# YannisLamp/crypto-recommendation

Hardware: AMD Instinct MI355X
Metric: point hash+assign ops/sec at d=128, N=10M, K=256; 1/2/4/8 MI355X (higher is better)
Workload: dtype fp32 points; split-f16 MFMA scores (f32 accumulate); tuples, bucket IDs and cluster IDs bit-exact (x87-exact hashing, certified argmin); distances: certified f32, <= 2^-20 relative to the reference's fp64 (north star: 1e-5; the context's default LSHKM_DIST_CERTIFIED mode), LSHKM_DIST_EXACT for the r; 1 GPU; C3 Lloyd K=256 + C2 LSH L=5 k=4 hashing, N=10000000 per GPU, d=128; N_per_gpu=10000000, N_total=10000000, d=128, K=256, L=5, k=4, nb=100000, parallelism=dp1 (row shards)

## Files before the change

### crypto-recommendation_amd/csrc/api.cpp

```cpp
#include <hip/hip_runtime.h>

#include <algorithm>
#include <cmath>
#include <cstring>
#include <map>
#include <mutex>
#include <random>
#include <sstream>
#include <string>
#include <vector>

#include "../../include/lshkm.h"
#include "common.h"
#include "kernels.h"
#include "index.h"

namespace lshkm {
static thread_local std::string g_err;
void set_error(const std::string& msg) { g_err = msg; }

int device_cu_count(int* ncu) {
    static std::mutex mu;
    static std::map<int, int> cus;
    int dev = 0;
// ... 551 lines not shown
    return lsh_hash_impl(lsh, X, N, tuples, phi, bucket);
}

int lshkm_lsh_hash_f64(lshkm_lsh lsh, const double* X, int64_t N, int32_t* tuples, int32_t* phi, int32_t* bucket) {
    return lsh_hash_impl(lsh, X, N, tuples, phi, bucket);
}

}

static int assign_path(int metric, int d, int K, bool f64) {
    if (test_switch("LSHKM_ASSIGN_PATH", "exact")) return 2;
    if (!test_switch("LSHKM_ASSIGN_PATH", "f32")) {
        const FusedRoute r = fused_route(metric != LSHKM_METRIC_EUCLIDEAN, f64, d, K, false, 0, 0,
                                         test_switch("LSHKM_FUSED_FORM", "chunked"));
        if (r.form != FusedForm::none) return r.rows == 0 ? 0 : 3;
    }
    return assign_dp(d) > 0 ? 1 : 2;
}

static bool fuse_hash(const lshkm_lsh_s* lsh, int metric, int K, bool f64) {
    const lshkm::ProjTable& pj = lsh->proj;
    if (lsh->metric != metric || !(metric == LSHKM_METRIC_EUCLIDEAN ? pj.fused_ok : pj.mfma_ok)) return false;
    return fused_route(metric != LSHKM_METRIC_EUCLIDEAN, f64, pj.d, K, true, pj.k, pj.LK,
                       test_switch("LSHKM_FUSED_FORM", "chunked")).form != FusedForm::none;
}

bool lshkm::exact_pruned(Pts X, int d, int K, int metric) {
    return K <= 1024 && d <= 256 && !test_switch("LSHKM_EXACT_PASS", "full") &&
           (metric == LSHKM_METRIC_EUCLIDEAN || !X.f64);
}

static size_t exact_ct_bytes(const AssignJob& q) { return (size_t)q.d * ((q.K + 255) / 256 * 256) * 8; }

int lshkm::exact_listed_prep(lshkm_ctx ctx, const AssignJob& q) {
    int rc;
    if ((rc = ctx->ws_ct.reserve(exact_ct_bytes(q)))) return rc;
    return launch_assign_pruned_prep(ctx->stream, q.X.f64, q.d, q.C, q.K, (float*)ctx->ws_ct.p,
                                     q.metric == LSHKM_METRIC_EUCLIDEAN ? 0 : 1);
}

int lshkm::exact_listed(lshkm_ctx ctx, const AssignJob& q, const RowList& l, bool exact_dist, bool prepped,
                        const double* xn2, const double* nbv) {
    const bool prune = exact_pruned(q.X, q.d, q.K, q.metric);
    if (!prune && (q.metric != LSHKM_METRIC_EUCLIDEAN || (l.nseg == 0 && q.d > 256)))
        return launch_assign_exact(ctx->stream, q, l, xn2, nbv);
    int rc;
    if ((rc = ctx->ws_ct.reserve(exact_ct_bytes(q)))) return rc;
    if (prune) return launch_assign_pruned_list(ctx->stream, q, (float*)ctx->ws_ct.p, l, exact_dist ? 1 : 0, prepped);
    return launch_assign_exact_list(ctx->stream, q, (double*)ctx->ws_ct.p, l);
}

static int assign_f32_mfma(lshkm_ctx ctx, const AssignJob& q) {
    hipStream_t s = ctx->stream;
    const int DP = assign_dp(q.d), Kpad = (q.K + 63) / 64 * 64;
    const int64_t N = q.N;
    int rc;
    if ((rc = ctx->ws_c32.reserve((size_t)Kpad * DP * 4)) || (rc = ctx->ws_cconst.reserve((size_t)3 * Kpad * 4)) ||
        (rc = ctx->ws_ambig.reserve((size_t)std::max<int64_t>(N, 1) * 2 * 4)) ||
        (rc = ctx->ws_counter.reserve(64)))
        return rc;
    unsigned long long* cnt = (unsigned long long*)ctx->ws_counter.p;
    LSHKM_HIP(hipMemsetAsync(cnt, 0, 16, s));
    if ((rc = launch_centroid_prep(s, q.C, q.K, Kpad, q.d, DP, q.metric, q.X.f64, (float*)ctx->ws_c32.p, (float*)ctx->ws_cconst.p))) return rc;
    if ((rc = launch_assign_mfma(s, q.X, N, q.d, DP, q.C, q.K, Kpad, q.metric, (const float*)ctx->ws_c32.p, (const float*)ctx->ws_cconst.p,
                                 q.assign, q.dist, (int32_t*)ctx->ws_ambig.p, cnt))) return rc;
    RowList l;
// ... 225 lines not shown
```

### crypto-recommendation_amd/csrc/fused.hip

```cpp
#include "../../include/lshkm.h"
#include "fused_impl.h"
#include "index.h"

namespace lshkm {

namespace {

struct FusedPlan {
    bool hash = false, cos = false;
    int rows = 0;
    int nblk = 0;
    int64_t seg_rows = 0;
    int np_hi = 0;
    int np_refine = 0;
};

int fused_workspace(lshkm_ctx ctx, const FusedShape& sh, FusedWorkspace& w) {
    const FusedLayout l = fused_layout(sh);
    int rc;
    struct { Buf& b; size_t bytes; } const bufs[] = {
        {ctx->ws_c32, l.c16},      {ctx->ws_cconst, l.cconst}, {ctx->ws_ambig, l.list1}, {ctx->ws_counter, l.counter},
        {ctx->ws_seg, l.seg1},     {ctx->ws_hfix, l.fix},      {ctx->ws_seg3, l.seg3},   {ctx->ws_part, l.part},
        {ctx->ws_ambig2, l.list2}, {ctx->ws_seg2, l.seg2},     {ctx->ws_tuples, l.tuples}, {ctx->ws_cf32, l.cf32},
        {ctx->ws_c64p, l.c64p},    {ctx->ws_xn2, l.xn2}};
    for (const auto& e : bufs)
        if (e.bytes && (rc = e.b.reserve(e.bytes))) return rc;
    const auto at = [](const Buf& b, size_t off) { return off == FusedLayout::NONE ? nullptr : (char*)b.p + off; };
    w.list_cap = l.list_cap;
    w.Ch = (_Float16*)at(ctx->ws_c32, 0); w.Cl = (_Float16*)at(ctx->ws_c32, l.cl_off);
    w.cbound = (float*)at(ctx->ws_cconst, 0); w.cnh = (float*)at(ctx->ws_cconst, l.cnh_off);
    w.nbv = (double*)at(ctx->ws_cconst, l.nbv_off);
    if (l.cf32) { w.C32 = (float*)at(ctx->ws_cf32, 0); w.rn32 = (float*)at(ctx->ws_cf32, l.rn32_off); }
    if (l.c64p) w.C64p = ctx->ws_c64p.as<double>();
    w.list1 = ctx->ws_ambig.as<int32_t>(); w.seg1 = ctx->ws_seg.as<int32_t>();
    w.list2 = ctx->ws_ambig2.as<int32_t>(); w.seg2 = ctx->ws_seg2.as<int32_t>();
    if (l.seg3) w.seg3 = ctx->ws_seg3.as<int32_t>();
    w.hfix = (unsigned long long*)at(ctx->ws_hfix, l.hfix_off);
    w.cfix = (unsigned long long*)at(ctx->ws_hfix, l.cfix_off);
    w.hfix2 = (unsigned long long*)at(ctx->ws_hfix, l.hfix2_off);
    if (l.part) w.part = ctx->ws_part.as<float4>();
    w.cnt = ctx->ws_counter.as<unsigned long long>();
    if (l.xn2) w.xn2 = ctx->ws_xn2.as<double>();
    if (l.tuples) w.tuples = ctx->ws_tuples.as<int32_t>();
    return 0;
}

FusedArgs fused_common_args(lshkm_ctx ctx, const AssignRequest& q, const FusedShape& sh, const FusedWorkspace& w) {
    FusedArgs a{};
    a.X = q.X.f64 ? nullptr : q.X.f(); a.X64 = q.X.f64 ? q.X.d() : nullptr;
    a.N = q.N; a.d = q.d;
    a.xvec = sh.rows == 1 ? (a.d % 4 == 0 && ((uintptr_t)a.X & 15) == 0) : (a.d % 2 == 0 && ((uintptr_t)a.X64 & 15) == 0);
    a.Ch = w.Ch; a.Cl = w.Cl; a.cnh = w.cnh; a.cbound = w.cbound; a.Kpad = sh.Kpad();
    a.C64 = w.C64p ? w.C64p : q.C; a.Cd = q.C;
    a.C32 = w.C32; a.rn32 = w.rn32; a.fast_dist = sh.fast ? 1 : 0;
    a.assign = q.assign; a.dist = q.dist;
    a.stats = ctx->stats.as<unsigned long long>();
    a.nb = 1;
    if (q.lsh) {
        const ProjTable& pj = q.lsh->proj;
        a.Vh = pj.vh_d.as<_Float16>(); a.Vl = pj.vl_d.as<_Float16>(); a.PT = pj.PT_d.as<double>();
        a.tv = pj.t_d.as<float>(); a.pnorm = pj.pn_d.as<double>(); a.v1 = pj.v1_d.as<double>();
        a.rv = pj.r_d.as<int32_t>(); a.w = pj.w; a.L = pj.L; a.k = pj.k; a.LK = pj.LK; a.LKpad = pj.LKpad;
        a.nb = q.lsh->nb;
    }
    a.bdiv = make_bucket_div(a.nb);
    if (sh.cosine) { a.nbv = w.nbv; a.xn2 = w.xn2; }
    a.cfix = w.cfix; a.cfix_counts = w.seg3; a.cfix_count = w.cfix ? w.cnt + CNT_CFIX : nullptr;
    a.pass_first = 1; a.pass_last = 1;
    return a;
}

void hash_outputs(FusedArgs& a, const AssignRequest& q, const FusedShape& sh, const FusedWorkspace& w) {
    a.hfix = w.hfix; a.hfix_count = w.hfix ? w.cnt + CNT_HFIX : nullptr;
    if (!q.lsh) return;
    a.phi = q.phi; a.bucket = q.bucket;
    a.tuples = sh.cosine ? nullptr : q.tuples ? q.tuples : w.tuples;
}

template <typename T>
// ... 69 lines not shown
            c->tev_side = true;
        }
        if (hipEventRecord(c->join_ev, c->side_stream) != hipSuccess) return kstatus("fused_assign (join)");
        return 0;
    }
    int join() {
        if (!open) return 0;
        if (hipStreamWaitEvent(c->stream, c->join_ev, 0) != hipSuccess) return kstatus("fused_assign (join)");
        open = false;
        return 0;
    }
    ~SideFork() { if (open) (void)hipStreamSynchronize(c->side_stream); }
};

#ifdef LSHKM_PHASE_TIMING
struct PhaseReport {
    hipStream_t s;
    unsigned long long* d = nullptr;
    explicit PhaseReport(hipStream_t s_) : s(s_) {
        static unsigned long long* prof_d = nullptr;
        if (!prof_d) (void)hipMalloc(&prof_d, 64);
        (void)hipMemsetAsync(prof_d, 0, 64, s);
        d = prof_d;
    }
    ~PhaseReport() {
        unsigned long long v[6];
        (void)hipMemcpyAsync(v, d, 48, hipMemcpyDeviceToHost, s);
        (void)hipStreamSynchronize(s);
        fprintf(stderr, "PHASES %llu %llu %llu %llu %llu\n", v[0], v[1], v[2], v[3], v[4]);
    }
};
#endif

}

int fused_assign(lshkm_ctx ctx, const AssignRequest& q) {
    hipStream_t s = ctx->stream;
    const bool cosine = q.metric != LSHKM_METRIC_EUCLIDEAN;
    const ProjTable* pj = q.lsh ? &q.lsh->proj : nullptr;
    const FusedRoute route = fused_route(cosine, q.X.f64, q.d, q.K, pj != nullptr, pj ? pj->k : 0, pj ? pj->LK : 0,
                                         test_switch("LSHKM_FUSED_FORM", "chunked"));
    if (route.form == FusedForm::none || (pj && (q.lsh->metric != q.metric || !pj->mfma_ok))) {
        set_error("fused_assign: no fused form runs this shape (fused_route, fused_layout.h)");
        return LSHKM_ERR_ARG;
    }
    FusedShape sh;
    sh.N = q.N; sh.d = q.d; sh.K = q.K; sh.cosine = cosine; sh.rows = route.rows;
    sh.hash = pj != nullptr; sh.LK = pj ? pj->LK : 0;
    sh.fast = !cosine && sh.rows != 2 && !q.force_exact && ctx->dist_mode == LSHKM_DIST_CERTIFIED;
    sh.image32 = sh.fast || (!cosine && sh.rows != 2 && sh.Kpad() <= 256 && !test_switch("LSHKM_GATHER32", "0"));
    sh.own_tuples = sh.hash && !cosine && !q.tuples;
    const bool pwfix = sh.pwfix();
    int rc;
    FusedWorkspace w;
    if ((rc = fused_workspace(ctx, sh, w))) return rc;
    LSHKM_HIP(hipMemsetAsync(w.cnt, 0, FUSED_COUNTER_CLEAR, s));
    if (ctx->timing) LSHKM_HIP(hipEventRecord(ctx->tev[0], s));
    ctx->tev_side = false;
    if ((rc = launch_fused_prep(s, q.C, q.K, q.d, cosine ? 1 : 0, w))) return rc;
    const bool xprep = exact_pruned(q.X, q.d, q.K, q.metric);
    if (xprep && (rc = exact_listed_prep(ctx, q))) return rc;
    if (w.xn2 && (rc = launch_row_sumsq(s, q.X.d(), q.N, q.d, w.xn2))) return rc;

    const FusedArgs common = fused_common_args(ctx, q, sh, w);
    RowList exact_rows;
    exact_rows.p = w.list1; exact_rows.count = w.cnt + CNT_AMBIG; exact_rows.bound = q.N;
    RecList dist_fix[2];
    int ndist_fix = 0;
    SideFork side{ctx};
    if (q.N > 0 && route.form == FusedForm::chunked) {
        FusedArgs a = common;
        hash_outputs(a, q, sh, w);
        a.ambig = w.list1; a.ambig_count = w.cnt + CNT_AMBIG;
        if ((rc = launch_fused_chunked(s, sh.hash, a))) return rc;
    } else if (q.N > 0) {
        FusedPlan p;
        p.hash = sh.hash; p.cos = cosine; p.rows = sh.rows;
        int ncu = 0;
        if (device_cu_count(&ncu)) return LSHKM_ERR_HIP;
        p.nblk = fused_grid(q.N, ncu);
        p.seg_rows = fused_seg_rows(q.N, p.nblk);
        if (p.nblk > FUSED_MAX_SEGS) {
            set_error("fused_assign: more blocks than list segments");
            return LSHKM_ERR_ARG;
        }
        p.np_hi = (sh.Kpad() + FH_KMAX - 1) / FH_KMAX;
        p.np_refine = (sh.Kpad() + FP_KMAX - 1) / FP_KMAX;
        const RowList l1 = segmented(w.list1, w.cnt + CNT_REFINED, w.seg1, q, p);
        const RecList lh = segmented(w.hfix, w.cnt + CNT_HFIX, w.seg1, q, p);
        const RowList l2 = segmented(w.list2, w.cnt + CNT_AMBIG, w.seg2, q, p);
        FusedArgs seg = common;
        seg.seg_rows = p.seg_rows; seg.part = w.part;
#ifdef LSHKM_PHASE_TIMING
        PhaseReport report(s);
        seg.prof = report.d;
#endif
        FusedArgs hi = seg;
        hash_outputs(hi, q, sh, w);
        hi.ambig = l1.p; hi.ambig_count = l1.count; hi.seg_counts = l1.counts;
        if ((rc = fused_hi_passes(s, hi, p))) return rc;
        if (sh.hash) {
            const bool forked = ctx->side_init() == 0;
            if (forked && (rc = side.fork())) return rc;
            launch_hash_fixup(forked ? ctx->side_stream : s, lh, cosine, hi);
            if (forked && (rc = side.end_side())) return rc;
        }
        FusedArgs rf = seg;
        rf.list_in = l1.p; rf.list_counts = l1.counts; rf.list_seg_rows = l1.seg_rows;
        rf.ambig = l2.p; rf.ambig_count = l2.count; rf.seg_counts = l2.counts;
        rf.hfix = cosine ? w.hfix2 : hi.hfix; rf.hfix_count = cosine ? w.cnt + CNT_CFIX : hi.hfix_count;
        if ((rc = fused_refine_passes(s, rf, p))) return rc;
        if (cosine && (rc = side.join())) return rc;
        if ((rc = kstatus("fused_hi_kernel"))) return rc;
        exact_rows = l2;
        if (cosine || pwfix) dist_fix[ndist_fix++] = segmented(w.cfix, w.cnt + CNT_CFIX, w.seg3, q, p);
        if (cosine) dist_fix[ndist_fix++] = segmented(w.hfix2, w.cnt + CNT_CFIX, w.seg2, q, p);
    }
    if (ctx->timing) LSHKM_HIP(hipEventRecord(ctx->tev[1], s));
    if ((rc = exact_listed(ctx, q, exact_rows, !sh.fast, xprep, cosine ? w.xn2 : nullptr, cosine ? w.nbv : nullptr)))
        return rc;
    if ((rc = side.join())) return rc;
    {
        int di[3], n = 0;
        const unsigned long long* sp[3];
        di[n] = STAT_REFINED; sp[n++] = w.cnt + CNT_REFINED;
        if (sh.hash) { di[n] = STAT_HASH_FIX; sp[n++] = w.cnt + CNT_HFIX; }
        di[n] = STAT_ASSIGN_AMBIG; sp[n++] = w.cnt + CNT_AMBIG;
        if ((rc = launch_add_counters(s, ctx->stats.as<unsigned long long>(), n, di, sp))) return rc;
    }
    if (cosine || pwfix) {
        if ((rc = launch_cos_fix_seg(s, q, ndist_fix, dist_fix, cosine ? w.xn2 : nullptr, cosine ? w.nbv : nullptr)))
            return rc;
        if ((rc = launch_add_counter(s, ctx->stats.as<unsigned long long>() + (cosine ? STAT_COS_FIX : STAT_POW_FIX),
                                     w.cnt + CNT_CFIX)))
            return rc;
    }
    return 0;
}

}
```

### crypto-recommendation_amd/csrc/fused_hi.hip

```cpp
#include "fused_impl.h"

namespace lshkm {

__host__ __device__ constexpr int fh_lds_bytes(int Kpad, bool hash) {
    return 16 + Kpad * FU_RS * 2 + Kpad * 4 + (hash ? 2 * 32 * FU_RS * 2 + FP_HC_BYTES : 0);
}
static_assert(fh_lds_bytes(FH_KMAX, true) <= 160 * 1024, "hi-only LDS image exceeds 160 KiB");
constexpr double FH_A = 130.0 * 0x1p-23;

constexpr int FH_WAVES_MPFAST = 12;
constexpr int FH_FAST_WAVES = 8;
template <bool HASH, bool MP, int MET, bool FAST = false>
__host__ __device__ constexpr int fh_waves() {
    return HASH && MP ? 12 : (MP && FAST ? FH_WAVES_MPFAST : (FAST && !MP ? FH_FAST_WAVES : 8));
}

__device__ inline int cosine_halves_finish(double sh0, double sl0, double ts0, double sh, double sl, double ts,
                                           double xa, double nbv, double& v) {
    const double mb = 2.0 * sqrt(__dmul_rn(xa, nbv)) * (1.0 + 0x1p-40);
    const double tsum = __dadd_rn(ts0, ts);
    if (!(tsum >= 0x1p-790)) return 2;
    IpAcc ip;
    const double t = __dadd_rn(sh0, sh);
    const double bb = __dsub_rn(t, sh0);
// ... 118 lines not shown
}

#ifndef LSHKM_ROWPF
#define LSHKM_ROWPF 3
#endif
constexpr int FH_ROWPF = LSHKM_ROWPF;
constexpr int FH_ROWPF_KMAX = 256;
constexpr int FH_ROWPF_WAVE = 32 * 64 * 4;
__host__ __device__ constexpr int fh_rowpf_off(int Kpad, bool hash) { return (fh_lds_bytes(Kpad, hash) + 255) & ~255; }
static_assert(fh_rowpf_off(FH_ROWPF_KMAX, true) + FH_FAST_WAVES * FH_ROWPF_WAVE <= 160 * 1024,
              "row prefetch buffers exceed 160 KiB");
static_assert(FH_ROWPF_KMAX <= FH_GATH_KMAX, "the FAST single-pass form runs where the gather ring would (fused.hip)");

__device__ inline void glds16s(const void* sbase, uint32_t voff, uint32_t lds_base, int lds_off) {
    unsigned keep;
    asm volatile("s_mov_b32 %0, m0\n\ts_add_u32 m0, %3, %4\n\ts_nop 0\n\tglobal_load_lds_dwordx4 %1, %2\n\ts_mov_b32 m0, %0"
                 : "=&s"(keep) : "v"(voff), "s"(sbase), "s"(lds_base), "n"(lds_off) : "memory", "scc");
}

template <bool HASH, bool MP = false, int MET = 0, int NIMG = 1, bool GATH = false, int ROWS = 0, bool FAST = false,
          int PF = 0, int HG = 4>
__global__ __launch_bounds__((64 * fh_waves<HASH, MP, MET, FAST>()), 1) void fused_hi_kernel(FusedArgs a) {
    constexpr int FH_WAVES = fh_waves<HASH, MP, MET, FAST>();
    constexpr int FH_THREADS = 64 * FH_WAVES;
    static_assert(NIMG == 1 || (!MP && MET == 0), "two-image form: euclidean, single launch");
    static_assert(!GATH || (!MP && MET == 0 && NIMG == 1 && FH_WAVES == 8), "gather ring: euclidean single pass");
    static_assert(ROWS == 0 || (!HASH && !MP && NIMG == 1), "general rows: Lloyd without hashing, one pass");
    static_assert(!(GATH && ROWS == 2), "fp64 rows re-read x in the chain: register loads of the winner rows");
    static_assert(!FAST || (MET == 0 && ROWS != 2 && NIMG == 1 && !GATH), "fast distance: euclidean, fp32 rows");
    static_assert(PF == 0 || (FAST && !MP && ROWS == 0 && FH_WAVES == FH_FAST_WAVES), "row prefetch: the FAST single-pass form");
    static_assert(HG == 4 || (HASH && MET == 0 && PF != 0 && HG >= 1 && HG < 4), "fewer live hash groups: the prefetching FAST form");
    constexpr bool PFR = (PF & 1) != 0, PFL = (PF & 2) != 0;
    extern __shared__ __attribute__((aligned(16))) char smem[];
    const int Kpad = a.Kpad;
    const bool fastd = FAST || a.fast_dist != 0;
    const int KI = NIMG == 2 ? FH_KMAX : Kpad;
    int* lcount = reinterpret_cast<int*>(smem);
    _Float16* lch = reinterpret_cast<_Float16*>(smem + 16);
    float* lcn = reinterpret_cast<float*>(lch + KI * FU_RS);
    _Float16* lvh = reinterpret_cast<_Float16*>(lcn + KI);
    _Float16* lvl = lvh + 32 * FU_RS;
    float* lpn0 = reinterpret_cast<float*>(lvl + 32 * FU_RS);
    float* lv10 = lpn0 + 32;
    float* lt0 = lv10 + 32;
    int32_t* lr0 = reinterpret_cast<int32_t*>(lt0 + 32);

    auto load_image = [&](int img) {
        const int r0 = img * KI, nr = NIMG == 2 && img == 1 ? Kpad - FH_KMAX : KI;
        constexpr int FH_CU = 8;
        for (int e0 = 0; e0 < nr * 16; e0 += FH_THREADS * FH_CU) {
            float4 v[FH_CU];
#pragma unroll
            for (int u = 0; u < FH_CU; u++) {
                const int e = e0 + u * FH_THREADS + (int)threadIdx.x < nr * 16 ? e0 + u * FH_THREADS + (int)threadIdx.x : 0;
                v[u] = *reinterpret_cast<const float4*>(a.Ch + (size_t)(r0 + (e >> 4)) * FU_D + (e & 15) * 8);
            }
#pragma unroll
            for (int u = 0; u < FH_CU; u++) {
                const int e = e0 + u * FH_THREADS + (int)threadIdx.x < nr * 16 ? e0 + u * FH_THREADS + (int)threadIdx.x : 0;
                *reinterpret_cast<float4*>(lch + (e >> 4) * FU_RS + (e & 15) * 8) = v[u];
            }
        }
        for (int e = threadIdx.x; e < nr; e += FH_THREADS) lcn[e] = a.cnh[r0 + e];
    };
    load_image(0);
    if (threadIdx.x < 3) lcount[threadIdx.x] = 0;
// ... 516 lines not shown
                }
                acc = take_from_upper(acc);
            }
            const bool pw_hard = pwl == nullptr && (pw.hard() || (ROWS != 2 && (__float_as_uint(a.cbound[7]) & 2u) != 0u));
            const int pw_other = __shfl_xor((int)pw_hard, 32);
            const bool hard = pw_hard || pw_other != 0;
            if (h == 1 && valid && cert) {
                a.assign[row] = I1;
                if (!hard) a.dist[row] = sqrt(acc);
            }
            const unsigned long long pb = __ballot(h == 1 && valid && cert && hard);
            if (pb) {
                const int leader = __builtin_ctzll(pb);
                int base = 0;
                if (lane == leader) base = atomicAdd(lcount + 2, __popcll(pb));
                base = __shfl(base, leader);
                if (h == 1 && valid && cert && hard) cfix_seg[base + __popcll(pb & ((1ull << lane) - 1ull))] = (unsigned long long)row;
            }
            __builtin_amdgcn_s_setprio(0);
        }
        PT_MARK(2)
    };
    if constexpr (PFR) {
        for (int64_t tile = tfirst + wave; tile < ntiles; tile += 2 * tstride) {
            tile_body(tile, xua, xub);
            if (tile + tstride >= ntiles) break;
            tile_body(tile + tstride, xub, xua);
        }
    } else {
        for (int64_t tile = tfirst + wave; NIMG == 2 ? rd < nround : tile < ntiles; tile += tstride, rd++)
            tile_body(tile, xua, xub);
    }
    PT_FLUSH
    __syncthreads();
    if (threadIdx.x < 2 && (!MP || (threadIdx.x == 0 ? (!HASH && a.pass_last != 0) : (HASH && a.pass_first)))) {
        const int c = lcount[threadIdx.x];
        a.seg_counts[SEG_SLOTS * blockIdx.x + threadIdx.x] = c;
        if (c) atomicAdd(threadIdx.x == 0 ? a.ambig_count : a.hfix_count, (unsigned long long)c);
    }
    if ((MET == 1 || !fastd) && threadIdx.x == 2 && (!MP || (!HASH && a.pass_last))) {
        const int c = lcount[2];
        a.cfix_counts[SEG_SLOTS * blockIdx.x + SEG_FIX] = c;
        if (c) atomicAdd(a.cfix_count, (unsigned long long)c);
    }
}

template <bool HASH, bool MP, int MET, int NIMG, bool GATH, int ROWS, bool FAST, int PF, int HG>
static void hi_launch(hipStream_t s, unsigned nblk, size_t lds, const FusedArgs& a) {
    hipLaunchKernelGGL((fused_hi_kernel<HASH, MP, MET, NIMG, GATH, ROWS, FAST, PF, HG>), dim3(nblk),
                       dim3(64 * fh_waves<HASH, MP, MET, FAST>()), lds, s, a);
}

int launch_fused_hi_pass(hipStream_t s, unsigned nblk, const HiForm& f, FusedArgs a) {
    size_t lds = (size_t)fh_lds_bytes(f.two_image ? FH_KMAX : a.Kpad, f.hash);
    a.pw_lds = 0;
    if (f.gath) {
        if (a.Kpad > FH_GATH_KMAX) {
            set_error("launch_fused_hi_pass: the gather ring needs K <= 256");
            return -1;
        }
        lds = (size_t)fh_gath_off(a.Kpad, f.hash) + 8 * FH_GATH_WAVE;
    } else if (f.rows == 2 && f.metric == 0) {
        constexpr int PW_BYTES = fh_waves<false, false, 0>() * 512 * 8;
        const size_t off = (lds + 255) & ~(size_t)255;
        if (off + PW_BYTES <= 160 * 1024) {
            a.pw_lds = (int)off;
// ... 54 lines not shown
```

### crypto-recommendation_amd/csrc/fused_impl.h

```cpp
#pragma once
#include <algorithm>
#include <cstdlib>
#include <cstring>
#include <cstdio>
#include <type_traits>

#include "common.h"
#include "kernels.h"
#include "hash_exact.h"
#include "exact.h"
#include "hash_tile.h"
#include "fused_args.h"

namespace lshkm {

static_assert(FU_D == FUSED_DIMS, "fused_layout.h states the kernels' dimension");
constexpr int FP_THREADS = 64 * FP_WAVES;
constexpr int FH_GATH_KMAX = 256;
constexpr int FP_HC_BYTES = 32 * (4 + 4 + 4 + 4);
constexpr int MFMA_PRIO = 1;
constexpr int CHAIN_PRIO = 2;

struct FusedWorkspace {
    int64_t list_cap = 0;
    _Float16 *Ch = nullptr, *Cl = nullptr;
    float *cbound = nullptr, *cnh = nullptr;
    double* nbv = nullptr;
    float *C32 = nullptr, *rn32 = nullptr;
    double* C64p = nullptr;
    int32_t *list1 = nullptr, *seg1 = nullptr;
    int32_t *list2 = nullptr, *seg2 = nullptr;
    int32_t* seg3 = nullptr;
    unsigned long long *hfix = nullptr, *cfix = nullptr, *hfix2 = nullptr;
    float4* part = nullptr;
    unsigned long long* cnt = nullptr;
    double* xn2 = nullptr;
    int32_t* tuples = nullptr;
};

int launch_fused_prep(hipStream_t s, const double* C, int K, int d, int metric, const FusedWorkspace& w);
int launch_row_sumsq(hipStream_t s, const double* X, int64_t N, int d, double* out);
int launch_fused_chunked(hipStream_t s, bool hash, const FusedArgs& a);
struct HiForm {
    bool hash = false;
    bool mp = false;
    int metric = 0;
    bool two_image = false;
    bool gath = false;
    int rows = 0;
    bool fast = false;
    bool rowpf = false;
};
int launch_fused_hi_pass(hipStream_t s, unsigned nblk, const HiForm& f, FusedArgs a);
int launch_fused_refine_pass(hipStream_t s, unsigned nblk, int metric, bool mp, int rows, const FusedArgs& a);
void launch_hash_fixup(hipStream_t s, const RecList& l, bool cosine, FusedArgs a);
int launch_cos_fix_seg(hipStream_t s, const AssignJob& q, int nlists, const RecList* lists, const double* xn2,
                       const double* nbv);

#ifdef LSHKM_PHASE_TIMING
#define PT_DECL unsigned long long pt_acc[6] = {0, 0, 0, 0, 0, 0}; unsigned long long pt_t = __builtin_amdgcn_s_memtime();
#define PT_MARK(i) { const unsigned long long t_ = __builtin_amdgcn_s_memtime(); pt_acc[i] += t_ - pt_t; pt_t = t_; }
#define PT_FLUSH if (lane == 0) for (int i_ = 0; i_ < 6; i_++) atomicAdd(a.prof + i_, pt_acc[i_]);
#elif defined(LSHKM_ISA_MARK)
#define PT_DECL
#define PT_MARK(i) asm volatile(";PTMARK " #i);
#define PT_FLUSH
#else
#define PT_DECL
#define PT_MARK(i)
#define PT_FLUSH
#endif

__device__ inline double swap_halves(double v, int h) {
// ... 102 lines not shown
```

### crypto-recommendation_amd/csrc/fused_layout.h

```cpp
#pragma once
#include <algorithm>
#include <cstddef>
#include <cstdint>

namespace lshkm {

constexpr int FP_WAVES = 8;
constexpr int FH_WAVES_MIN = 8, FH_WAVES_MAX = 12;
constexpr int HMF_W = 4;
constexpr int HMF_BPC = 2;
constexpr int FP_KMAX = 256;
constexpr int FH_KMAX = 512;
constexpr int FUSED_DIMS = 128;

enum class FusedForm { none, hi, chunked };
struct FusedRoute {
    FusedForm form;
    int rows;
};
inline FusedRoute fused_route(bool cosine, bool f64, int d, int K, bool hash, int k, int LK, bool chunked_switch) {
    const bool hash_ok = !hash || (LK >= 1 && LK <= 32 && (!cosine || k == 4));
    if (!f64 && d == FUSED_DIMS && hash_ok) {
        if (!cosine) return {chunked_switch || (hash && k != 4) ? FusedForm::chunked : FusedForm::hi, 0};
        if (!chunked_switch) return {FusedForm::hi, 0};
// ... 7 lines not shown
constexpr size_t SEG_COUNTER_BYTES = (size_t)FUSED_MAX_SEGS * SEG_SLOTS * 4;
constexpr int64_t FUSED_LIST_SLACK = 32 + (int64_t)FUSED_MAX_SEGS * FH_WAVES_MAX * 32;
inline int64_t fused_list_cap(int64_t N) { return N + FUSED_LIST_SLACK; }
inline int64_t seg_rows_for(int64_t N, int nblk, int W) {
    const int64_t ntiles = (N + 31) / 32;
    return (int64_t)W * 32 * ((ntiles + (int64_t)nblk * W - 1) / ((int64_t)nblk * W));
}
inline int fused_grid(int64_t N, int ncu) {
    const int64_t want = ((N + 31) / 32 + FP_WAVES - 1) / FP_WAVES;
    return (int)std::max<int64_t>(1, std::min<int64_t>(ncu, want));
}
inline int64_t fused_seg_rows(int64_t N, int nblk) {
    int64_t r = 0;
    for (const int W : {FP_WAVES, FH_WAVES_MIN, FH_WAVES_MAX}) r = std::max(r, seg_rows_for(N, nblk, W));
    return r;
}
inline int hash_mfma_grid(int64_t N, int ncu) {
    const int64_t want = ((N + 31) / 32 + HMF_W - 1) / HMF_W;
    return (int)std::max<int64_t>(1, std::min<int64_t>((int64_t)ncu * HMF_BPC, want));
}
inline int64_t hash_mfma_seg_rows(int64_t N, int nblk) { return seg_rows_for(N, nblk, HMF_W); }

constexpr int64_t FUSED_PART_BYTES_PER_ROW = 32;
inline int64_t fused_part_bytes(int64_t N) {
    const int64_t tiles = std::max<int64_t>((N + 31) / 32, (fused_list_cap(N) + 31) / 32 + FUSED_MAX_SEGS);
    return tiles * 32 * FUSED_PART_BYTES_PER_ROW;
}

constexpr int CNT_AMBIG = 0;
constexpr int CNT_HFIX = 1;
constexpr int CNT_REFINED = 2;
constexpr int CNT_CFIX = 3;
constexpr size_t FUSED_COUNTER_BYTES = 64, FUSED_COUNTER_CLEAR = 32;

struct FusedShape {
    int64_t N = 0;
    int d = FUSED_DIMS, K = 0;
    bool cosine = false;
    int rows = 0;
    bool hash = false;
    int LK = 0;
    bool fast = false;
    bool image32 = false;
    bool own_tuples = false;
    int Kpad() const { return (K + 63) / 64 * 64; }
    bool pwfix() const { return !cosine && !fast; }
};
struct FusedLayout {
    static constexpr size_t NONE = ~(size_t)0;
    int64_t list_cap = 0;
    int64_t part_bytes = 0;
    size_t c16 = 0;
    size_t cconst = 0;
    size_t list1 = 0, list2 = 0;
    size_t seg1 = 0, seg2 = 0, seg3 = 0;
    size_t counter = 0;
    size_t fix = 0;
    size_t part = 0;
    size_t tuples = 0;
    size_t cf32 = 0;
    size_t c64p = 0;
    size_t xn2 = 0;
    size_t cl_off = 0, cnh_off = 0, nbv_off = 0, rn32_off = 0;
    size_t hfix_off = NONE, cfix_off = NONE, hfix2_off = NONE;
};
inline FusedLayout fused_layout(const FusedShape& q) {
// ... 46 lines not shown
```

### crypto-recommendation_amd/csrc/fused_small.hip

```cpp
#include "fused_impl.h"

namespace lshkm {

constexpr int HF_WAVES = 4;
constexpr int HF_SPLIT = 4;
constexpr int HF_G = 8;
constexpr int HF_SLOTS = 64 * HF_WAVES / HF_G;
constexpr int HF_XL = FU_D / HF_G;
constexpr int HF_PS = 33;
constexpr int HF_QS = HF_XL * HF_PS + 4;
constexpr size_t HF_LDS = (size_t)HF_G * HF_QS * 8 + 32 * (8 + 8 + 4);
__device__ inline int hf_pidx(int r) { return ((r >> 2) & 7) * HF_QS + (((r >> 5) << 2) | (r & 3)) * HF_PS; }

template <int CTRL>
__device__ inline uint32_t dpp_move(uint32_t v) {
    return (uint32_t)__builtin_amdgcn_mov_dpp((int)v, CTRL, 0xF, 0xF, false);
}
template <int CTRL>
__device__ inline double dpp_move(double v) {
    const uint64_t b = (uint64_t)__double_as_longlong(v);
    const uint64_t lo = dpp_move<CTRL>((uint32_t)b), hi = dpp_move<CTRL>((uint32_t)(b >> 32));
    return __longlong_as_double((long long)((hi << 32) | lo));
}
template <int CTRL>
// ... 253 lines not shown
            const double up = 1.0 + 0x1p-18;
            const double nc = sqrt(s2) * (1.0 + 0x1p-30);
            m[0] = __float_as_uint((float)((FU_A1 + 0x1p-22) * nc * up));
            m[1] = __float_as_uint((float)((FU_A2 * s1 * (1.0 + 0x1p-20) + (metric == 1 ? 0.0 : 0x1p-23 * s2) +
                                            0x1p-41 * s2) * up));
            m[2] = anybad ? 1u : 0u;
            m[3] = __float_as_uint((float)(nc * up));
            m[4] = __float_as_uint((float)(sqrt(rr) * (1.0 + 0x1p-30) * up));
            m[5] = __float_as_uint((float)(sqrt(hh) * (1.0 + 0x1p-30) * up));
            m[6] = __float_as_uint((float)(metric == 1 ? 0.0 : 0.5 * s2 * up));
        }
#pragma unroll
        for (int i = 0; i < 8; i++) wmax[threadIdx.x >> 6][i] = m[i];
    }
    __syncthreads();
    if (threadIdx.x < 8) {
        const int i = threadIdx.x;
        unsigned int v = 0u;
        for (int w = 0; w < FP_PREP_WAVES; w++) v = i == 2 || i == 7 ? (v | wmax[w][i]) : max(v, wmax[w][i]);
        if (v) {
            if (i == 2 || i == 7) atomicOr(cb + i, v);
            else atomicMax(cb + i, v);
        }
    }
}

int launch_fused_prep(hipStream_t s, const double* C, int K, int d, int metric, const FusedWorkspace& w) {
    const int Kpad = (K + 63) / 64 * 64;
    static_assert(64 % FP_PREP_WAVES == 0, "Kpad is a multiple of 64");
    (void)hipMemsetAsync(w.cbound, 0, 32, s);
    hipLaunchKernelGGL(fused_centroid_prep, dim3((unsigned)(Kpad / FP_PREP_WAVES)), dim3(64 * FP_PREP_WAVES), 0, s, C, K, Kpad, w.Ch, w.Cl, w.cnh,
                       reinterpret_cast<unsigned int*>(w.cbound), metric, w.nbv, w.C32, w.rn32, d, w.C64p);
    return kstatus("fused_centroid_prep");
}

constexpr int CF_SPLIT = 8;
struct CosLists {
    const unsigned long long* list[2];
    const int32_t* counts[2];
};
template <typename TX, int MET>
__global__ __launch_bounds__(256) void cos_fix_seg_kernel(const TX* __restrict__ X, int d, const double* __restrict__ C,
                                                          CosLists cl, int nseg, int64_t seg_rows,
                                                          const int32_t* __restrict__ assign, double* __restrict__ dist,
                                                          const double* __restrict__ xn2, const double* __restrict__ nbv) {
    const int per_list = nseg * CF_SPLIT;
    const int li = blockIdx.x / per_list, b = blockIdx.x % per_list;
    const int seg = b % nseg, part = b / nseg;
    const int n = cl.counts[li][SEG_SLOTS * seg + SEG_FIX];
    const unsigned long long* l = cl.list[li] + (int64_t)seg * seg_rows;
    const bool vec = sizeof(TX) == 4 && d % 8 == 0 && ((uintptr_t)X & 15) == 0 && ((uintptr_t)C & 15) == 0;
    __shared__ double sqs[4][64 * 16];
    double* sq = sqs[threadIdx.x >> 6];
    const int lane = threadIdx.x & 63;
    for (int i0 = part * 256 + (threadIdx.x & ~63); i0 < n; i0 += CF_SPLIT * 256) {
        const int i = i0 + lane;
        const bool live = i < n;
        const int64_t row = (int64_t)l[live ? i : i0];
        const TX* xr = X + row * d;
        const double* cr = C + (size_t)assign[row] * d;
        double v;
        if constexpr (MET == 1) {
            if (nbv && (sizeof(TX) == 4 || xn2)) {
                const double xa = sizeof(TX) == 4 ? -1.0 : xn2[row], cb = nbv[assign[row]];
                if (vec) v = exact_cosine_x87_pf<sizeof(TX) == 4>(xr, cr, d, xa, cb);
                else v = exact_cosine_x87_pf<false>(xr, cr, d, xa, cb);
// ... 114 lines not shown
```

### crypto-recommendation_amd/csrc/index.h

```cpp
#pragma once
#include <algorithm>
#include <hip/hip_runtime.h>
#include <stdint.h>

#include <vector>

#include "kernels.h"

namespace lshkm {

struct Buf {
    void* p = nullptr;
    size_t cap = 0;
    Buf() = default;
    Buf(const Buf&) = delete;
    Buf& operator=(const Buf&) = delete;
    ~Buf();
    int reserve(size_t bytes);
    template <typename T> T* as() const { return reinterpret_cast<T*>(p); }
};

struct ProjTable {
    int metric = 0, d = 0, L = 0, k = 0, LK = 0, LKpad = 0;
    float w = 0.f;
    Buf PT_d, t_d, pn_d, r_d;
    bool fused_ok = false;
    bool mfma_ok = false;
    Buf vh_d, vl_d, v1_d;
    std::vector<float> hV;
    int upload(hipStream_t s, int metric, int d, int L, int k, float w, const float* V, const float* t,
               const int32_t* r, const double* R);
    HashParams params(int64_t nb) const;
    HashMfmaParams mfma_params(int64_t nb) const;
};

}

struct lshkm_ctx_s;
struct lshkm_lsh_s;
namespace lshkm {
int hash_rows(lshkm_ctx_s* ctx, int mode, Pts X, int64_t N, const ProjTable& pj, int64_t nb, int32_t* out_h,
              int32_t* out_phi, int32_t* out_bucket, int32_t* mm, bool* h16 = nullptr);
bool exact_pruned(Pts X, int d, int K, int metric);
int exact_listed_prep(lshkm_ctx_s* ctx, const AssignJob& q);
int exact_listed(lshkm_ctx_s* ctx, const AssignJob& q, const RowList& l, bool exact_dist, bool prepped,
                 const double* xn2, const double* nbv);
struct AssignRequest : AssignJob {
    const ::lshkm_lsh_s* lsh = nullptr;
    int32_t *tuples = nullptr, *phi = nullptr, *bucket = nullptr;
    bool force_exact = false;
};
int fused_assign(lshkm_ctx_s* ctx, const AssignRequest& q);

}

struct lshkm_ctx_s {
    int device = 0;
    int dist_mode = 0;
    hipStream_t stream = nullptr;
    hipStream_t own_stream = nullptr;
    lshkm::Buf stats;
    lshkm::Buf ws_c32, ws_cconst, ws_ambig, ws_counter, ws_src, ws_hfix, ws_ct, ws_seg, ws_tuples, ws_part;
    lshkm::Buf ws_cf32, ws_c64p;
    lshkm::Buf ws_ambig2, ws_seg2;
    lshkm::Buf ws_seg3;
    lshkm::Buf ws_xn2;
    lshkm::Buf ws[16];
    lshkm::Buf ws_range[9];
    lshkm::Buf ws_sil_near;
    lshkm::Buf ws_sil_s;
    lshkm::Buf ws_long;
    lshkm::Buf ws_km;
    lshkm::Buf ws_km_seg;
    lshkm::Buf ws_scan;
    lshkm::Buf ws_pam[5];
    lshkm::Buf ws_call[10];
    lshkm::Buf ws_lshpc[7];
    uint64_t ws_epoch = 0;
    bool timing = false;
    hipEvent_t tev[3] = {nullptr, nullptr, nullptr};
    bool tev_side = false;
    hipStream_t side_stream = nullptr;
    hipEvent_t fork_ev = nullptr, join_ev = nullptr;
    int side_init() {
        if (side_stream) return 0;
        if (hipStreamCreateWithFlags(&side_stream, hipStreamNonBlocking) != hipSuccess) return -2;
        if (hipEventCreateWithFlags(&fork_ev, hipEventDisableTiming) != hipSuccess ||
            hipEventCreateWithFlags(&join_ev, hipEventDisableTiming) != hipSuccess)
            return -2;
        return 0;
    }
    static constexpr int PIN_SLOTS = 4;
    void* pin_buf[PIN_SLOTS] = {};
    size_t pin_cap[PIN_SLOTS] = {};
    hipEvent_t pin_ev[PIN_SLOTS] = {};
    bool pin_used[PIN_SLOTS] = {};
    int pin_cur = -1;
    void* pinned = nullptr;
    hipEvent_t pinned_ev = nullptr;
// ... 95 lines not shown
```

Before: 5.159 billion point hash+assign ops/s.

## Merge centroid prep, counter clear and exact-pruned prep into one kernel

Replaces the counter memset, the fused centroid prep kernel and the separate exact-listed prep kernel with a single merged prep kernel for Euclidean d=128 when K<=1024. The merged kernel derives the f16 split images, norms, bounds and the transposed f32 centroid table in one pass, combining per-block maxima through atomics and a last-block finalize. This removes several small launches and a memset from each assign call, at the cost of global atomics and a persistent zeroed scratch workspace. It also adds an optional per-wave span probe behind a compile flag and a test entry point.

```diff
diff --git a/crypto-recommendation_amd/csrc/api.cpp b/crypto-recommendation_amd/csrc/api.cpp
--- a/crypto-recommendation_amd/csrc/api.cpp
+++ b/crypto-recommendation_amd/csrc/api.cpp
@@ -607,6 +607,13 @@
 
 static size_t exact_ct_bytes(const AssignJob& q) { return (size_t)q.d * ((q.K + 255) / 256 * 256) * 8; }
 
+int lshkm::exact_listed_workspace(lshkm_ctx ctx, const AssignJob& q, float** ws) {
+    int rc;
+    if ((rc = ctx->ws_ct.reserve(exact_ct_bytes(q)))) return rc;
+    *ws = (float*)ctx->ws_ct.p;
+    return 0;
+}
+
 int lshkm::exact_listed_prep(lshkm_ctx ctx, const AssignJob& q) {
     int rc;
     if ((rc = ctx->ws_ct.reserve(exact_ct_bytes(q)))) return rc;
diff --git a/crypto-recommendation_amd/csrc/fused.hip b/crypto-recommendation_amd/csrc/fused.hip
--- a/crypto-recommendation_amd/csrc/fused.hip
+++ b/crypto-recommendation_amd/csrc/fused.hip
@@ -25,6 +25,15 @@
         {ctx->ws_c64p, l.c64p},    {ctx->ws_xn2, l.xn2}};
     for (const auto& e : bufs)
         if (e.bytes && (rc = e.b.reserve(e.bytes))) return rc;
+    if (!ctx->ws_prep.p) {
+        if ((rc = ctx->ws_prep.reserve(FUSED_PREP_BYTES))) return rc;
+        if (hipMemset(ctx->ws_prep.p, 0, FUSED_PREP_BYTES) != hipSuccess) {
+            (void)hipFree(ctx->ws_prep.p);
+            ctx->ws_prep.p = nullptr; ctx->ws_prep.cap = 0;
+            return kstatus("fused_assign (prep workspace)");
+        }
+    }
+    w.prep = ctx->ws_prep.as<unsigned int>();
     const auto at = [](const Buf& b, size_t off) { return off == FusedLayout::NONE ? nullptr : (char*)b.p + off; };
     w.list_cap = l.list_cap;
     w.Ch = (_Float16*)at(ctx->ws_c32, 0); w.Cl = (_Float16*)at(ctx->ws_c32, l.cl_off);
@@ -45,6 +54,20 @@
     return 0;
 }
 
+int fused_prepare(lshkm_ctx ctx, const AssignJob& q, bool cosine, bool xprep, const FusedWorkspace& w) {
+    hipStream_t s = ctx->stream;
+    int rc;
+    const bool merged = fused_prep_merged_covers(q.K, q.d, cosine ? 1 : 0, w) && !test_switch("LSHKM_PREP", "split");
+    float* xws = nullptr;
+    if (merged && xprep && (rc = exact_listed_workspace(ctx, q, &xws))) return rc;
+    if (!merged) LSHKM_HIP(hipMemsetAsync(w.cnt, 0, FUSED_COUNTER_CLEAR, s));
+    if (ctx->timing) LSHKM_HIP(hipEventRecord(ctx->tev[0], s));
+    ctx->tev_side = false;
+    if (merged) return launch_fused_prep_merged(s, q.C, q.K, q.X.f64, w, xws);
+    if ((rc = launch_fused_prep(s, q.C, q.K, q.d, cosine ? 1 : 0, w))) return rc;
+    return xprep ? exact_listed_prep(ctx, q) : 0;
+}
+
 FusedArgs fused_common_args(lshkm_ctx ctx, const AssignRequest& q, const FusedShape& sh, const FusedWorkspace& w) {
     FusedArgs a{};
     a.X = q.X.f64 ? nullptr : q.X.f(); a.X64 = q.X.f64 ? q.X.d() : nullptr;
@@ -180,6 +203,45 @@
 };
 #endif
 
+#ifdef LSHKM_WAVE_SPAN
+struct SpanReport {
+    static constexpr size_t WORDS = 2 * (size_t)FUSED_MAX_SEGS * FH_WAVES_MAX;
+    hipStream_t s;
+    unsigned long long* d = nullptr;
+    explicit SpanReport(hipStream_t s_) : s(s_) {
+        static unsigned long long* span_d = nullptr;
+        if (!span_d) (void)hipMalloc(&span_d, WORDS * 8);
+        if (span_d) (void)hipMemsetAsync(span_d, 0, WORDS * 8, s);
+        d = span_d;
+    }
+    ~SpanReport() {
+        if (!d) return;
+        std::vector<unsigned long long> v(WORDS);
+        if (hipMemcpyAsync(v.data(), d, WORDS * 8, hipMemcpyDeviceToHost, s) != hipSuccess ||
+            hipStreamSynchronize(s) != hipSuccess)
+            return;
+        std::vector<double> span, end;
+        unsigned long long t0 = ~0ull;
+        for (size_t i = 0; i < WORDS; i += 2)
+            if (v[i + 1]) t0 = std::min(t0, v[i]);
+        double sum = 0.0;
+        for (size_t i = 0; i < WORDS; i += 2)
+            if (v[i + 1]) {
+                sum += (double)(v[i + 1] - v[i]) * 0.01;
+                end.push_back((double)(v[i + 1] - t0) * 0.01);
+            }
+        if (end.empty()) return;
+        std::sort(end.begin(), end.end());
+        const size_t n = end.size();
+        const auto pct = [&](double q) { return end[std::min(n - 1, (size_t)(q * (double)n))]; };
+        double mean = 0.0;
+        for (const double e : end) mean += e / (double)n;
+        fprintf(stderr, "SPAN waves %zu kernel %.1f us residency %.3f end min %.1f p10 %.1f p50 %.1f mean %.1f p90 %.1f max %.1f us\n",
+                n, end[n - 1], sum / ((double)n * end[n - 1]), end[0], pct(0.1), pct(0.5), mean, pct(0.9), end[n - 1]);
+    }
+};
+#endif
+
 }
 
 int fused_assign(lshkm_ctx ctx, const AssignRequest& q) {
@@ -202,12 +264,8 @@
     int rc;
     FusedWorkspace w;
     if ((rc = fused_workspace(ctx, sh, w))) return rc;
-    LSHKM_HIP(hipMemsetAsync(w.cnt, 0, FUSED_COUNTER_CLEAR, s));
-    if (ctx->timing) LSHKM_HIP(hipEventRecord(ctx->tev[0], s));
-    ctx->tev_side = false;
-    if ((rc = launch_fused_prep(s, q.C, q.K, q.d, cosine ? 1 : 0, w))) return rc;
     const bool xprep = exact_pruned(q.X, q.d, q.K, q.metric);
-    if (xprep && (rc = exact_listed_prep(ctx, q))) return rc;
+    if ((rc = fused_prepare(ctx, q, cosine, xprep, w))) return rc;
     if (w.xn2 && (rc = launch_row_sumsq(s, q.X.d(), q.N, q.d, w.xn2))) return rc;
 
     const FusedArgs common = fused_common_args(ctx, q, sh, w);
@@ -242,6 +300,9 @@
 #ifdef LSHKM_PHASE_TIMING
         PhaseReport report(s);
         seg.prof = report.d;
+#elif defined(LSHKM_WAVE_SPAN)
+        SpanReport report(s);
+        seg.prof = report.d;
 #endif
         FusedArgs hi = seg;
         hash_outputs(hi, q, sh, w);
@@ -287,3 +348,37 @@
 }
 
 }
+
+#ifdef LSHKM_TEST_SWITCHES
+extern "C" int lshkm_test_fused_prep(lshkm_ctx ctx, const double* C, int K, int xf64, void* out, int64_t out_bytes,
+                                     int64_t* need) {
+    using namespace lshkm;
+    LSHKM_CHECK(ctx && C && need && K >= 1 && K <= 1024, LSHKM_ERR_ARG, "lshkm_test_fused_prep: bad argument");
+    hipStream_t s = ctx->stream;
+    AssignJob q;
+    q.X = xf64 ? Pts((const double*)nullptr) : Pts((const float*)nullptr);
+    q.N = 0; q.d = FU_D; q.C = C; q.K = K; q.metric = LSHKM_METRIC_EUCLIDEAN;
+    FusedShape sh;
+    sh.N = 0; sh.d = FU_D; sh.K = K; sh.rows = xf64 ? 2 : 0;
+    sh.fast = sh.image32 = !xf64;
+    const FusedLayout l = fused_layout(sh);
+    const size_t Kpad = (size_t)sh.Kpad(), cb = (Kpad + 8) * 4, xb = ((size_t)FU_D * Kpad + Kpad + Kpad / 32) * 4;
+    *need = (int64_t)(l.c16 + cb + l.cf32 + FUSED_COUNTER_CLEAR + xb);
+    if (!out || out_bytes < *need) return 0;
+    int rc;
+    FusedWorkspace w;
+    float* xws = nullptr;
+    if ((rc = fused_workspace(ctx, sh, w)) || (rc = exact_listed_workspace(ctx, q, &xws))) return rc;
+    struct { void* p; size_t bytes; } const parts[] = {
+        {w.Ch, l.c16}, {w.cbound, cb}, {w.C32, l.cf32}, {w.cnt, FUSED_COUNTER_CLEAR}, {xws, xb}};
+    for (const auto& e : parts)
+        if (e.bytes) LSHKM_HIP(hipMemsetAsync(e.p, 0xA5, e.bytes, s));
+    if ((rc = fused_prepare(ctx, q, false, true, w))) return rc;
+    char* o = (char*)out;
+    for (const auto& e : parts) {
+        if (e.bytes) LSHKM_HIP(hipMemcpyAsync(o, e.p, e.bytes, hipMemcpyDeviceToDevice, s));
+        o += e.bytes;
+    }
+    return 0;
+}
+#endif
diff --git a/crypto-recommendation_amd/csrc/fused_hi.hip b/crypto-recommendation_amd/csrc/fused_hi.hip
--- a/crypto-recommendation_amd/csrc/fused_hi.hip
+++ b/crypto-recommendation_amd/csrc/fused_hi.hip
@@ -174,6 +174,9 @@
     static_assert(HG == 4 || (HASH && MET == 0 && PF != 0 && HG >= 1 && HG < 4), "fewer live hash groups: the prefetching FAST form");
     constexpr bool PFR = (PF & 1) != 0, PFL = (PF & 2) != 0;
     extern __shared__ __attribute__((aligned(16))) char smem[];
+#ifdef LSHKM_WAVE_SPAN
+    const unsigned long long span_t0 = __builtin_amdgcn_s_memrealtime();
+#endif
     const int Kpad = a.Kpad;
     const bool fastd = FAST || a.fast_dist != 0;
     const int KI = NIMG == 2 ? FH_KMAX : Kpad;
@@ -756,6 +759,13 @@
             tile_body(tile, xua, xub);
     }
     PT_FLUSH
+#ifdef LSHKM_WAVE_SPAN
+    if (a.prof && lane == 0) {
+        unsigned long long* sp = a.prof + 2 * ((size_t)blockIdx.x * FH_WAVES + (threadIdx.x >> 6));
+        sp[0] = span_t0;
+        sp[1] = __builtin_amdgcn_s_memrealtime();
+    }
+#endif
     __syncthreads();
     if (threadIdx.x < 2 && (!MP || (threadIdx.x == 0 ? (!HASH && a.pass_last != 0) : (HASH && a.pass_first)))) {
         const int c = lcount[threadIdx.x];
diff --git a/crypto-recommendation_amd/csrc/fused_impl.h b/crypto-recommendation_amd/csrc/fused_impl.h
--- a/crypto-recommendation_amd/csrc/fused_impl.h
+++ b/crypto-recommendation_amd/csrc/fused_impl.h
@@ -34,11 +34,14 @@
     unsigned long long *hfix = nullptr, *cfix = nullptr, *hfix2 = nullptr;
     float4* part = nullptr;
     unsigned long long* cnt = nullptr;
+    unsigned int* prep = nullptr;
     double* xn2 = nullptr;
     int32_t* tuples = nullptr;
 };
 
 int launch_fused_prep(hipStream_t s, const double* C, int K, int d, int metric, const FusedWorkspace& w);
+bool fused_prep_merged_covers(int K, int d, int metric, const FusedWorkspace& w);
+int launch_fused_prep_merged(hipStream_t s, const double* C, int K, bool xf64, const FusedWorkspace& w, float* xws);
 int launch_row_sumsq(hipStream_t s, const double* X, int64_t N, int d, double* out);
 int launch_fused_chunked(hipStream_t s, bool hash, const FusedArgs& a);
 struct HiForm {
diff --git a/crypto-recommendation_amd/csrc/fused_layout.h b/crypto-recommendation_amd/csrc/fused_layout.h
--- a/crypto-recommendation_amd/csrc/fused_layout.h
+++ b/crypto-recommendation_amd/csrc/fused_layout.h
@@ -63,6 +63,9 @@
 constexpr int CNT_REFINED = 2;
 constexpr int CNT_CFIX = 3;
 constexpr size_t FUSED_COUNTER_BYTES = 64, FUSED_COUNTER_CLEAR = 32;
+constexpr int FUSED_PREP_CHUNKS = 16;
+constexpr int FUSED_PREP_BOUNDS = 0, FUSED_PREP_CHUNK = 8, FUSED_PREP_DONE = FUSED_PREP_CHUNK + 2 * FUSED_PREP_CHUNKS;
+constexpr size_t FUSED_PREP_BYTES = ((size_t)FUSED_PREP_DONE + 8) * 4;
 
 struct FusedShape {
     int64_t N = 0;
diff --git a/crypto-recommendation_amd/csrc/fused_small.hip b/crypto-recommendation_amd/csrc/fused_small.hip
--- a/crypto-recommendation_amd/csrc/fused_small.hip
+++ b/crypto-recommendation_amd/csrc/fused_small.hip
@@ -309,6 +309,162 @@
     hipLaunchKernelGGL(fused_centroid_prep, dim3((unsigned)(Kpad / FP_PREP_WAVES)), dim3(64 * FP_PREP_WAVES), 0, s, C, K, Kpad, w.Ch, w.Cl, w.cnh,
                        reinterpret_cast<unsigned int*>(w.cbound), metric, w.nbv, w.C32, w.rn32, d, w.C64p);
     return kstatus("fused_centroid_prep");
+}
+
+constexpr int MP_KMAX = 1024;
+constexpr int MP_WAVES = 8;
+constexpr int MP_TS = FU_D + 1;
+static_assert(64 % MP_WAVES == 0, "a block lies within one chunk");
+static_assert(MP_KMAX / 64 <= FUSED_PREP_CHUNKS, "two words of w.prep per chunk");
+
+struct PrepSums {
+    double s2, s1, rr, hh, r32;
+    bool bad, not32, tiny;
+    float f[2];
+    _Float16 h[2], l[2];
+};
+__device__ inline PrepSums prep_sums(const double (&raw)[2], bool real) {
+    PrepSums p;
+    p.s2 = p.s1 = p.rr = p.hh = p.r32 = 0.0;
+    bool bad = false, not32 = false, tiny = false;
+#pragma unroll
+    for (int u = 0; u < 2; u++) {
+        const double v = raw[u];
+        const float f = (float)v;
+        not32 |= real && (double)f != v;
+        tiny |= real && fabs(v) < 0x1p-460 && v != 0.0;
+        const double e = v - (double)f;
+        p.r32 = fma(e, e, p.r32);
+        const _Float16 hv = (_Float16)f;
+        p.f[u] = f; p.h[u] = hv; p.l[u] = (_Float16)(f - (float)hv);
+        p.s2 = fma(v, v, p.s2);
+        p.s1 += fabs(v);
+        const double r = v - (double)hv;
+        p.rr = fma(r, r, p.rr);
+        p.hh = fma((double)hv, (double)hv, p.hh);
+        bad |= !(fabs(v) <= (double)FU_RANGE);
+    }
+    for (int off = 32; off >= 1; off >>= 1) {
+        p.s2 += __shfl_xor(p.s2, off);
+        p.s1 += __shfl_xor(p.s1, off);
+        p.rr += __shfl_xor(p.rr, off);
+        p.hh += __shfl_xor(p.hh, off);
+        p.r32 += __shfl_xor(p.r32, off);
+    }
+    p.bad = __ballot(bad) != 0ull;
+    p.not32 = __ballot(not32) != 0ull;
+    p.tiny = __ballot(tiny) != 0ull;
+    return p;
+}
+
+struct MergedPrep {
+    const double* C;
+    int K, Kpad, xf64;
+    _Float16 *Ch, *Cl;
+    float *cnh, *C32, *rn32;
+    unsigned int* cb;
+    unsigned int* prep;
+    unsigned long long* cnt;
+    float* xws;
+};
+
+__global__ __launch_bounds__(64 * MP_WAVES) void fused_prep_merged(MergedPrep a) {
+    __shared__ float tile[MP_WAVES * MP_TS];
+    __shared__ unsigned int wmax[MP_WAVES][10];
+    __shared__ int last;
+    const int lane = threadIdx.x & 63, wave = threadIdx.x >> 6;
+    const int K = a.K, Kpad = a.Kpad;
+    const int cbase = MP_WAVES * (int)blockIdx.x, c = cbase + wave, chunk = cbase / 64;
+    if (blockIdx.x == 0 && threadIdx.x < FUSED_COUNTER_CLEAR / 8) a.cnt[threadIdx.x] = 0ull;
+    double raw[2];
+    {
+        const int cc = min(c, K - 1);
+        const double r0 = a.C[(size_t)cc * FU_D + lane], r1 = a.C[(size_t)cc * FU_D + lane + 64];
+        raw[0] = c < K ? r0 : 0.0;
+        raw[1] = c < K ? r1 : 0.0;
+    }
+    const PrepSums p = prep_sums(raw, c < K);
+    tile[wave * MP_TS + lane] = p.f[0];
+    tile[wave * MP_TS + lane + 64] = p.f[1];
+    unsigned int m[10] = {0u, 0u, 0u, 0u, 0u, 0u, 0u, 0u, 0u, 0u};
+    if (c < K) {
+        const double s2 = p.s2, s1 = p.s1;
+        const double up = 1.0 + 0x1p-18;
+        const double nc = sqrt(s2) * (1.0 + 0x1p-30);
+        m[0] = __float_as_uint((float)((FU_A1 + 0x1p-22) * nc * up));
+        m[1] = __float_as_uint((float)((FU_A2 * s1 * (1.0 + 0x1p-20) + 0x1p-23 * s2 + 0x1p-41 * s2) * up));
+        m[2] = p.bad ? 1u : 0u;
+        m[3] = __float_as_uint((float)(nc * up));
+        m[4] = __float_as_uint((float)(sqrt(p.rr) * (1.0 + 0x1p-30) * up));
+        m[5] = __float_as_uint((float)(sqrt(p.hh) * (1.0 + 0x1p-30) * up));
+        m[6] = __float_as_uint((float)(0.5 * s2 * up));
+        m[7] = (p.not32 ? 1u : 0u) | (p.tiny ? 2u : 0u);
+        const int d = FU_D;
+        const double sq = s2;
+        const double ec = 0x1p-24 * (2.0 * d + 12.0 + (a.xf64 ? 2.0 : 0.0)) * nc * up;
+        const double eb = (0x1p-24 * 5.0 * sq + 0x1p-40 * sq + (a.xf64 ? 0x1p-140 * nc : 0.0)) * up + 1e-30;
+        m[8] = __float_as_uint((float)(ec * (1.0 + 0x1p-20)));
+        m[9] = __float_as_uint((float)(eb * (1.0 + 0x1p-20)));
+    }
+    if (lane == 0) {
+#pragma unroll
+        for (int i = 0; i < 10; i++) wmax[wave][i] = m[i];
+    }
+    __syncthreads();
+    if (threadIdx.x < 10) {
+        const int i = threadIdx.x;
+        const bool bits = i == 2 || i == 7;
+        unsigned int v = 0u;
+        for (int w = 0; w < MP_WAVES; w++) v = bits ? (v | wmax[w][i]) : max(v, wmax[w][i]);
+        unsigned int* dst = a.prep + (i < 8 ? FUSED_PREP_BOUNDS + i : FUSED_PREP_CHUNK + 2 * chunk + (i - 8));
+        unsigned int old = 0u;
+        if (v) old = bits ? atomicOr(dst, v) : atomicMax(dst, v);
+        asm volatile("s_waitcnt vmcnt(0)" : : "v"(old) : "memory");
+    }
+    __syncthreads();
+    if (threadIdx.x == 0)
+        last = __hip_atomic_fetch_add(a.prep + FUSED_PREP_DONE, 1u, __ATOMIC_RELAXED, __HIP_MEMORY_SCOPE_AGENT) == gridDim.x - 1;
+#pragma unroll
+    for (int u = 0; u < 2; u++) {
+        const size_t o = (size_t)c * FU_D + lane + 64 * u;
+        if (a.C32) a.C32[o] = p.f[u];
+        a.Ch[o] = p.h[u];
+        a.Cl[o] = p.l[u];
+    }
+    float* CT32 = a.xws;
+    float* cn2 = a.xws ? a.xws + (size_t)FU_D * Kpad : nullptr;
+    if (lane == 0) {
+        if (a.rn32) a.rn32[c] = p.r32 == 0.0 ? 0.f : (float)(sqrt(p.r32) * (1.0 + 0x1p-40)) * (1.f + 0x1p-22f);
+        a.cnh[c] = c < K ? (float)(-0.5 * p.s2) : -0x1p100f;
+        if (cn2) cn2[c] = c < K ? (float)p.s2 : __builtin_inff();
+    }
+    if (CT32) {
+        const int cl = threadIdx.x % MP_WAVES;
+        for (int j = threadIdx.x / MP_WAVES; j < FU_D; j += 64) CT32[(size_t)j * Kpad + cbase + cl] = tile[cl * MP_TS + j];
+    }
+    __syncthreads();
+    if (!last) return;
+    const int nch = Kpad / 64;
+    if (threadIdx.x < 8 + 2 * nch) {
+        const int i = threadIdx.x;
+        const unsigned int v = atomicExch(a.prep + (i < 8 ? FUSED_PREP_BOUNDS + i : FUSED_PREP_CHUNK + (i - 8)), 0u);
+        if (i < 8) a.cb[i] = v;
+        else if (cn2) reinterpret_cast<unsigned int*>(cn2 + Kpad)[i - 8] = v;
+    }
+    if (threadIdx.x == 0) __hip_atomic_store(a.prep + FUSED_PREP_DONE, 0u, __ATOMIC_RELAXED, __HIP_MEMORY_SCOPE_AGENT);
+}
+
+bool fused_prep_merged_covers(int K, int d, int metric, const FusedWorkspace& w) {
+    return metric == 0 && d == FU_D && !w.C64p && K >= 1 && (K + 63) / 64 * 64 <= MP_KMAX;
+}
+
+int launch_fused_prep_merged(hipStream_t s, const double* C, int K, bool xf64, const FusedWorkspace& w, float* xws) {
+    MergedPrep a;
+    a.C = C; a.K = K; a.Kpad = (K + 63) / 64 * 64; a.xf64 = xf64 ? 1 : 0;
+    a.Ch = w.Ch; a.Cl = w.Cl; a.cnh = w.cnh; a.C32 = w.C32; a.rn32 = w.rn32;
+    a.cb = reinterpret_cast<unsigned int*>(w.cbound); a.prep = w.prep; a.cnt = w.cnt; a.xws = xws;
+    hipLaunchKernelGGL(fused_prep_merged, dim3((unsigned)(a.Kpad / MP_WAVES)), dim3(64 * MP_WAVES), 0, s, a);
+    return kstatus("fused_prep_merged");
 }
 
 constexpr int CF_SPLIT = 8;
diff --git a/crypto-recommendation_amd/csrc/index.h b/crypto-recommendation_amd/csrc/index.h
--- a/crypto-recommendation_amd/csrc/index.h
+++ b/crypto-recommendation_amd/csrc/index.h
@@ -43,6 +43,7 @@
               int32_t* out_phi, int32_t* out_bucket, int32_t* mm, bool* h16 = nullptr);
 bool exact_pruned(Pts X, int d, int K, int metric);
 int exact_listed_prep(lshkm_ctx_s* ctx, const AssignJob& q);
+int exact_listed_workspace(lshkm_ctx_s* ctx, const AssignJob& q, float** ws);
 int exact_listed(lshkm_ctx_s* ctx, const AssignJob& q, const RowList& l, bool exact_dist, bool prepped,
                  const double* xn2, const double* nbv);
 struct AssignRequest : AssignJob {
@@ -65,6 +66,7 @@
     lshkm::Buf ws_ambig2, ws_seg2;
     lshkm::Buf ws_seg3;
     lshkm::Buf ws_xn2;
+    lshkm::Buf ws_prep;
     lshkm::Buf ws[16];
     lshkm::Buf ws_range[9];
     lshkm::Buf ws_sil_near;
```

After: 5.207 billion point hash+assign ops/s, median of 6. Within noise of the previous version (+0.9%).
